# hsinnan75/MapCaller

Measured on AMD Instinct MI355X. Metric: reads/sec (150 bp PE vs GRCh38) at 1/2/4/8 MI355X; SAM CIGAR bit-exact, higher is better.
Workload: dtype u64/int32; 1 GPU; synthetic GRCh38-sized genome, 3100 Mbp (synthetic: GRCh38 is unavailable offline; repeat landscape in the detail record), 4000000 pairs x 150 bp PE per step per GPU (sub 0.005, ins 0.001, del 0.001 per base), -alg ksw2

## Files before the change

mapcaller_amd/csrc/mcx_ctx.h:

```cpp
#ifndef MCX_CTX_H
#define MCX_CTX_H
#include <hip/hip_runtime.h>
#include <algorithm>
#include <atomic>
#include <chrono>
#include <cmath>
#include <cstdio>
#include <cstdlib>
#include <cstring>
#include <string>
#include <type_traits>
#include <vector>

#include "../../include/mcx.h"
#include "mcx_dp.h"
#include "mcx_dp_lane2.h"
#include "mcx_simple.h"
#include "mcx_profile.h"
#include "mcx_internal.h"

using namespace mcx;

#define HIP_TRY(expr)                                                                                  \
    do {                                                                                               \
        hipError_t e_ = (expr);                                                                        \
        if (e_ != hipSuccess)                                                                          \
            return mcx_set_error(MCX_ERR_DEVICE, std::string(#expr) + ": " + hipGetErrorString(e_));   \
    } while (0)

template <typename F>
static inline hipError_t timed_wait(bool on, const char *what, int line, F &&f)
{
    if (!on) return f();
    const auto t0 = std::chrono::steady_clock::now();
    const hipError_t e = f();
    const double ms = std::chrono::duration<double, std::milli>(std::chrono::steady_clock::now() - t0).count();
    if (ms > 15) fprintf(stderr, "[mcx] %.1f ms in %s (line %d)\n", ms, what, line);
    return e;
}
extern std::atomic<size_t> g_dmalloc_bytes;
template <class T>
static int dmalloc(T **p, size_t n, int line = __builtin_LINE(), const char *file = __builtin_FILE())
{
    HIP_TRY(hipMalloc((void **)p, n * sizeof(T)));
    g_dmalloc_bytes += n * sizeof(T);
    static const bool log = getenv("MCX_ALLOC_LOG") != nullptr;
    if (log && n * sizeof(T) >= ((size_t)256 << 20)) fprintf(stderr, "[mcx alloc] %8.2f GB at %s:%d\n", (double)(n * sizeof(T)) / 1e9, file, line);
    return 0;
}

struct PairSel {
    const uint32_t *ids;
    const int32_t *est;
    uint32_t n;
};

static __device__ __forceinline__ uint32_t sel_pair(const PairSel &s, uint32_t local) { return s.ids ? s.ids[local] : local; }

constexpr int kCntPad = 64;
constexpr int kDpBuckets = 1024;

struct Knobs {
    bool timing = false, seed_one_base = false, dp_by_wave = false, dp_lane_always = false, late_reseed = false, no_work_order = false, no_simple = false,
         simple_no_dp = false, cluster_by_lane = false, rescue_in_line = false, build_by_lane = false, no_sums_cache = false, prof_by_column = false,
         tier1_hist = false, dp_hist = false, no_tier_overlap = false, no_late_overlap = false, no_prof_overlap = false, no_prepack = false, no_tier1_grow = false;
    int seed_fm_budget = 6, build_wave_limit = 0x7fffffff;
    uint32_t order_min = 16384u;
};

struct Tier {
    Caps caps;
    Layout lay;
    uint8_t *state = nullptr;
    uint32_t max_pairs = 0;
    uint32_t grow_to = 0;
};

enum { CNT_TASKS = 0, CNT_RESCUE = 1 * kCntPad, CNT_JOB0 = 2 * kCntPad, CNT_JOB1 = 3 * kCntPad, CNT_JOB2 = 4 * kCntPad, CNT_JOB3 = 5 * kCntPad,
       CNT_JOB4 = 6 * kCntPad, CNT_JOB5 = 7 * kCntPad, CNT_OV = 8 * kCntPad, CNT_LF = 9 * kCntPad, CNT_CELLS = 10 * kCntPad, CNT_UNSUP = 11 * kCntPad,
       CNT_QUEUE = 12 * kCntPad, CNT_EARLY = 13 * kCntPad, CNT_LATE = 14 * kCntPad, CNT_RTASK = 15 * kCntPad, CNT_RPLAN = 16 * kCntPad, CNT_RESCUE_N = 17 * kCntPad, CNT_RSEED = 18 * kCntPad,
       CNT_SIMPLE = 19 * kCntPad, CNT_EARLY_HITS = 20 * kCntPad, CNT_SIMPLE_LATER = 21 * kCntPad, CNT_SIMPLE_JOBS = 22 * kCntPad, CNT_N = 23 * kCntPad,
       CNT_ORDER = CNT_N, CNT_DP_SORT = CNT_ORDER + 16 * kCntPad, CNT_ALL = CNT_DP_SORT + 4 * kDpBuckets };
constexpr uint32_t kLateRoom = 2048;

struct RescueTask; struct RescueRes; struct RescuePlan;
struct PassRes {
    hipStream_t stream = nullptr;
    uint32_t *d_cnt = nullptr, *h_cnt = nullptr;
    uint2 *d_tasks = nullptr; uint32_t task_cap = 0;
    DpJob *d_jobs[kDpClasses] = {nullptr, nullptr, nullptr, nullptr, nullptr, nullptr}; uint32_t job_cap[kDpClasses] = {0, 0, 0, 0, 0, 0};
    uint32_t *d_rescue = nullptr; uint32_t rescue_cap = 0;
    uint32_t *d_kscratch = nullptr;
    RescueTask *d_rtasks = nullptr; RescueRes *d_rres = nullptr; Hit *d_rseeds = nullptr; RescuePlan *d_rplans = nullptr; uint32_t *d_rescue_n = nullptr;
    uint32_t rtask_cap = 0, rseed_cap = 0;
    uint8_t *d_dp_scratch[3] = {nullptr, nullptr, nullptr}; uint64_t dp_stride[3] = {0, 0, 0}; uint32_t dp_blocks[3] = {0, 0, 0};
    uint32_t *d_dp_lane = nullptr; uint32_t dp_lane_blocks = 0;
    uint32_t *d_dp_order[2] = {nullptr, nullptr};
    hipStream_t dp_stream[5] = {nullptr, nullptr, nullptr, nullptr, nullptr}; hipEvent_t dp_fork = nullptr, dp_join[5] = {nullptr, nullptr, nullptr, nullptr, nullptr};
    uint32_t *d_ov = nullptr; uint32_t ov_cap = 0;
    uint32_t *d_sel_ids = nullptr; int32_t *d_est = nullptr;
    hipEvent_t ev[12] = {nullptr, nullptr, nullptr, nullptr, nullptr, nullptr, nullptr, nullptr, nullptr, nullptr, nullptr, nullptr};
};

struct BatchRun {
    bool open = false, sums_valid = false, keys_out = false;
    ReadBatch rb; int paired = 0;
    uint32_t n_pairs = 0, n_chunks = 0, longest = 0;
    AlnRec *recs = nullptr; uint32_t *cig = nullptr;
    uint32_t cig_cap = 0, cig_words = 0;
    int64_t read_base = 0, mapped = 0;
    unsigned long long hs[3] = {0, 0, 0};
    std::vector<uint32_t> ok, ds;
    const uint32_t *d_ok = nullptr, *d_ds = nullptr;
    const uint64_t *d_sorted_keys = nullptr; uint64_t n_keys = 0; uint32_t n_sparse_keys = 0;
    std::chrono::steady_clock::time_point t0, t_begun; double ms_setup = 0;
    mcx_stats *stats = nullptr;
};
// ... 114 lines not shown
```

mapcaller_amd/csrc/mcx_pipeline.hip:

```cpp
#include "mcx_ctx.h"
#include <hipcub/hipcub.hpp>

static thread_local std::string g_err;
static int fail(int code, const std::string &msg) { g_err = msg; return code; }
int mcx_set_error(int code, const std::string &msg) { return fail(code, msg); }
extern "C" const char *mcx_last_error(void) { return g_err.c_str(); }
extern "C" int mcx_device_count(void)
{
    int n = 0;
    if (hipGetDeviceCount(&n) != hipSuccess) return 0;
    return n;
}

struct EndsLds { int64_t pos[kLdsEnds]; int32_t chr[kLdsEnds]; };

static __device__ __forceinline__ void stage_ends(IndexView &ix, EndsLds &l)
{
    if (ix.n_ends <= kLdsEnds) {
        for (int i = threadIdx.x; i < ix.n_ends; i += blockDim.x) { l.pos[i] = ix.end_pos[i]; l.chr[i] = ix.end_chr[i]; }
        __syncthreads();
        ix.end_pos = l.pos; ix.end_chr = l.chr;
    }
}

// ... 282 lines not shown
}

__global__ void __launch_bounds__(256) k_order_place(PairSel sel, const uint32_t *read_blocks, int nr, uint32_t *counts, uint32_t *order, const uint8_t *done)
{
    __shared__ uint32_t n_cls[kWorkClasses], at_cls[kWorkClasses];
    if (threadIdx.x < kWorkClasses) n_cls[threadIdx.x] = 0u;
    __syncthreads();
    const uint32_t base = blockIdx.x * (256u * kOrderTile);
    const int lane = threadIdx.x & 63;
    int cls[kOrderTile];
#pragma unroll
    for (int t = 0; t < kOrderTile; t++) {
        const uint32_t local = base + t * 256u + threadIdx.x;
        cls[t] = local < sel.n ? pair_work_class(sel, local, read_blocks, nr, done) : -1;
#pragma unroll
        for (int k = 0; k < kWorkClasses; k++) {
            const uint64_t m = __ballot(cls[t] == k);
            if (lane == 0 && m) atomicAdd(&n_cls[k], (uint32_t)__popcll(m));
        }
    }
    __syncthreads();
    if (threadIdx.x < kWorkClasses) {
        uint32_t first = 0;
        for (int k = 0; k < (int)threadIdx.x; k++) first += counts[k * kCntPad];
        const uint32_t mine = n_cls[threadIdx.x];
        at_cls[threadIdx.x] = first + (mine ? atomicAdd(counts + (8 + threadIdx.x) * kCntPad, mine) : 0u);
    }
    __syncthreads();
#pragma unroll
    for (int t = 0; t < kOrderTile; t++) {
        const uint32_t local = base + t * 256u + threadIdx.x;
#pragma unroll
        for (int k = 0; k < kWorkClasses; k++) {
            const uint64_t m = __ballot(cls[t] == k);
            uint32_t b = 0;
            if (lane == 0 && m) b = atomicAdd(&at_cls[k], (uint32_t)__popcll(m));
            b = __shfl(b, 0, 64);
            if (cls[t] == k) order[b + (uint32_t)__popcll(m & ((1ull << lane) - 1ull))] = local;
        }
    }
}

struct SimpleLater {
    uint32_t *pairs;
    SimpleJob *jobs;
    SimpleRes *res;
    uint32_t *job_list;
    uint32_t *n_pairs, *n_jobs;
    uint32_t cap;
};

template <bool NW, int MODE, bool DETAIL>
__global__ void __launch_bounds__(256) k_simple(Ctx cx, ReadBatch rb, uint32_t n_pairs, const int32_t *est, const uint32_t *read_blocks, AlnRec *recs, PairOut *pout,
                                                uint8_t *done, uint32_t *pool_over, uint32_t *n_done, SimpleLater sl)
{
    __shared__ EndsLds ends;
    __shared__ uint16_t cig_stage[256 * 2 * kSimpleRuns];
    __shared__ uint32_t job_stage[MODE == kDpCollect ? 3 * kSimpleJobs * 256 : 1];
    stage_ends(cx.ix, ends);
    const uint32_t slot = blockIdx.x * blockDim.x + threadIdx.x;
    const int nr = cx.pm.paired ? 2 : 1;
    uint16_t *stage = cig_stage + threadIdx.x;
    const uint32_t n_slots = MODE == kDpReplay ? min(*sl.n_pairs, sl.cap) : n_pairs;
    bool ok = slot < n_slots;
    const uint32_t pair = MODE == kDpReplay ? (ok ? sl.pairs[slot] : 0u) : slot;
    SimpleRead sr[2];
    int rl[2] = {0, 0};
    typename std::conditional<DETAIL, SimpleDetail, SimpleNoDetail>::type det;
    SimpleDpIo io;
    io.mode = MODE == kDpCollect && !sl.pairs ? kDpNone : MODE;
    io.jobs = MODE == kDpCollect ? job_stage + threadIdx.x : nullptr; io.job_stride = 256;
    io.res = MODE == kDpReplay ? sl.res + (uint64_t)slot * kSimpleJobs : nullptr;
    io.n = 0; io.read = 0;
    bool later = false;
    if (ok) {
        const PairState st = pair_state(cx.state, cx.lay, cx.caps, pair);
#pragma unroll
        for (int s = 0; s < 2; s++) {
            if (s < nr && ok) {
                const uint32_t r = pair * nr + s;
                const int nh = (int)(read_blocks[r] >> 20);
                rl[s] = (int)(rb.off[r + 1] - rb.off[r]);
                io.read = r;
                ok = nh >= 1 && nh <= kSimpleHits && !(cx.read_ext[r] >> 31);
                if (ok) {
                    if constexpr (DETAIL) { uint8_t *rec = cx.detail + (uint64_t)r * cx.dlay.stride; det.frags = (Frag *)(rec + sizeof(DetailHdr)); det.ops = rec + cx.dlay.off_ops; }
                    const int how = simple_read<NW, uint16_t>(cx.ix, cx.pm, rl[s], cx.packed + (uint64_t)r * cx.wpad, st.hits[s], nh, sr[s], stage + s * kSimpleRuns * 256, 256, io, det);
                    ok = how != kSimpleNo;
                    later = later || how == kSimpleLater;
                }
            }
        }
        if (ok && nr == 2) ok = simple_pair_ok(sr[0], sr[1], est[pair]);
    }
    if (MODE == kDpCollect) {
        const bool wait = ok && later;
        const uint32_t at = wave_reserve(sl.n_pairs, wait ? 1u : 0u);
        const bool kept = wait && at < sl.cap;
        const uint32_t jat = wave_reserve(sl.n_jobs, kept ? (uint32_t)io.n : 0u);
        if (kept) {
            sl.pairs[at] = pair;
            for (int k = 0; k < io.n; k++) {
                const uint32_t *w = job_stage + (3 * k) * 256 + threadIdx.x;
                sl.jobs[(uint64_t)at * kSimpleJobs + k] = simple_job_unpack(w[0], w[256], w[512], pair * (uint32_t)nr, nr);
                sl.job_list[jat + k] = at * kSimpleJobs + (uint32_t)k;
            }
            done[pair] = 2;
        }
        if (wait) ok = false;
        later = kept;
    }
    const uint32_t want = ok ? (uint32_t)sr[0].n_cig + (nr == 2 ? (uint32_t)sr[1].n_cig : 0u) : 0u;
    const uint32_t at = wave_reserve(cx.cig_pool_n, want);
    const uint64_t took = __ballot(ok);
    if ((threadIdx.x & 63) == 0 && took) atomicAdd(n_done, (uint32_t)__popcll(took));
    if (slot >= n_slots) return;
    if (ok && at + want > cx.cig_pool_cap) { atomicOr(pool_over, 1u); ok = false; }
    if (!later) done[pair] = ok ? 1 : 0;
    if (!ok) return;
    const uint32_t off[2] = {at, at + (uint32_t)sr[0].n_cig};
#pragma unroll
    for (int s = 0; s < 2; s++) {
        if (s >= nr) break;
        for (int k = 0; k < sr[s].n_cig; k++) cx.cig_pool[off[s] + k] = (uint32_t)stage[(s * kSimpleRuns + k) * 256];
    }
    AlnRec rec2[2];
    PairOut po;
    simple_pair(cx, nr == 2, sr[0], sr[nr - 1], rl[0], rl[nr - 1], est[pair], rec2, off, po);
    recs[(uint64_t)pair * nr] = rec2[0];
    if (nr == 2) recs[(uint64_t)pair * nr + 1] = rec2[1];
    pout[pair] = po;
    if constexpr (DETAIL) {
#pragma unroll
        for (int s = 0; s < 2; s++) {
            if (s >= nr) break;
            const DetailHdr d = simple_detail_hdr(cx.ix, nr == 2, s, sr[0], sr[nr - 1]);
            *(DetailHdr *)(cx.detail + ((uint64_t)pair * nr + s) * cx.dlay.stride) = d;
        }
    }
}

template <bool NW>
__global__ void __launch_bounds__(256) k_simple_dp(Ctx cx, SimpleLater sl)
{
    constexpr int W = 2 + kSimpleDp * LaneDir<16, NW>::words;
    __shared__ uint32_t words[W * 256];
    const uint32_t n = min(*sl.n_jobs, sl.cap * kSimpleJobs);
    LaneMem mem; mem.base = words; mem.stride = 256; mem.lane = threadIdx.x;
    for (uint32_t i = blockIdx.x * blockDim.x + threadIdx.x; i < n; i += gridDim.x * blockDim.x) {
        const uint32_t at = sl.job_list[i];
        const SimpleJob j = sl.jobs[at];
        sl.res[at] = simple_dp_job<NW>(cx.ix, j, cx.packed + (uint64_t)j.read * cx.wpad, mem);
    }
}

static __device__ __forceinline__ uint32_t listed_pairs(const PairSel &sel, const uint32_t *order_cnt)
{
    if (!order_cnt) return sel.n;
    uint32_t n = 0;
#pragma unroll
    for (int k = 0; k < kWorkClasses; k++) n += order_cnt[k * kCntPad];
    return n;
}

__global__ void __launch_bounds__(256) k_cluster(Ctx cx, ReadBatch rb, PairSel sel, RescueList rl, const uint32_t *read_blocks, EarlyList el, const uint32_t *order,
                                                 const uint32_t *order_cnt, int cls_lo, int cls_hi)
{
    __shared__ EndsLds ends;
    uint32_t first = 0, n_listed = listed_pairs(sel, order_cnt);
    if (order_cnt && order) {
        uint32_t at = 0;
        for (int k = 0; k < kWorkClasses; k++) { if (k == cls_lo) first = at; at += order_cnt[k * kCntPad]; if (k == cls_hi) n_listed = at; }
    }
    if (first + blockIdx.x * blockDim.x >= n_listed) return;
    stage_ends(cx.ix, ends);
    const uint32_t slot = first + blockIdx.x * blockDim.x + threadIdx.x;
    const bool in = slot < n_listed;
    const uint32_t local = in ? (order ? order[slot] : slot) : 0u;
    uint32_t need = 0, over = 0;
    if (in) {
        ReadRef rd[2];
// ... 678 lines not shown
    int n_cig[2] = {0, 0};
    uint8_t *detail2 = nullptr;
    if (active) {
        pair = sel_pair(sel, local);
        make_reads(cx, rb, pair, rd);
        st = pair_state(cx.state, cx.lay, cx.caps, local);
        h = *st.hdr;
        st.hdr = &h;
        detail2 = cx.detail ? cx.detail + (int64_t)pair * nr * cx.dlay.stride : nullptr;
        finish_scores(cx, st, rd, (DetailHdr *)detail2, n_cig, nullptr, stage, 256);
    }
    const uint32_t want = (uint32_t)(n_cig[0] + n_cig[1]);
    const uint32_t at = wave_reserve(cx.cig_pool_n, want);
    const bool own = active && !(h.flags & (kDispatched | kOvAny));
    int n_ext[2] = {0, 0}, n_extw[2] = {0, 0};
    uint32_t at_ext = 0, at_extw = 0;
    if (kMulti) {
        if (own) for (int s = 0; s < nr; s++) n_ext[s] = extra_lines(st, s, rd, &n_extw[s]);
        at_ext = wave_reserve(mo.cnt, (uint32_t)(n_ext[0] + n_ext[1]));
        at_extw = wave_reserve(mo.cnt + 1, (uint32_t)(n_extw[0] + n_extw[1]));
    }
    if (!active || (h.flags & kDispatched)) return;
    const bool fits = at + want <= cx.cig_pool_cap;
    if (!fits) atomicOr(pool_over, 1u);
    const uint32_t off[2] = {at, at + (uint32_t)n_cig[0]};
    finish_records(cx, st, rd, recs + (int64_t)pair * nr, fits ? cx.cig_pool : nullptr, off, n_cig, detail2, stage, 256);
    if (kMulti && own) {
        const bool room = at_ext + (uint32_t)(n_ext[0] + n_ext[1]) <= mo.rec_cap && at_extw + (uint32_t)(n_extw[0] + n_extw[1]) <= mo.word_cap;
        for (int s = 0; s < nr; s++) {
            const uint32_t ro = at_ext + (s ? (uint32_t)n_ext[0] : 0u), wo = at_extw + (s ? (uint32_t)n_extw[0] : 0u);
            mo.ref[(int64_t)pair * nr + s] = room || n_ext[0] + n_ext[1] == 0 ? make_uint4(ro, (uint32_t)n_ext[s], wo, (uint32_t)n_extw[s]) : make_uint4(0u, (uint32_t)n_ext[s] | kMxOver, 0u, 0u);
            if (room && n_ext[s]) emit_extra(cx, st, s, rd, mo.recs + ro, mo.cig + wo, wo);
        }
    }
    PairOut o;
    o.flags = h.flags; o.est = h.est; o.est_lo = h.est_lo; o.est_hi = h.est_hi;
    o.pair_dist = h.pair_dist; o.pair_ok = (int16_t)h.pair_ok; o.mapped = (int16_t)h.mapped;
    pout[pair] = o;
    if (h.flags & kOvAny) {
        const uint32_t at2 = atomicAdd(n_ov, 1u);
        if (at2 < ov_cap) ov_ids[at2] = pair;
    }
}

static Knobs knobs_read()
{
    Knobs k;
    auto on = [](const char *name) { return getenv(name) != nullptr; };
    k.timing = on("MCX_TIMING"); k.seed_one_base = on("MCX_SEED_ONE_BASE"); k.dp_by_wave = on("MCX_DP_BY_WAVE"); k.dp_lane_always = on("MCX_DP_LANE_ALWAYS");
    k.late_reseed = on("MCX_LATE_RESEED"); k.no_work_order = on("MCX_NO_WORK_ORDER"); k.no_simple = on("MCX_NO_SIMPLE"); k.simple_no_dp = on("MCX_SIMPLE_NO_DP");
    k.cluster_by_lane = on("MCX_CLUSTER_BY_LANE"); k.rescue_in_line = on("MCX_RESCUE_IN_LINE"); k.build_by_lane = on("MCX_BUILD_BY_LANE");
    k.no_sums_cache = on("MCX_NO_SUMS_CACHE"); k.prof_by_column = on("MCX_PROF_BY_COLUMN"); k.tier1_hist = on("MCX_TIER1_HIST"); k.dp_hist = on("MCX_DP_HIST");
    k.no_tier_overlap = on("MCX_NO_TIER_OVERLAP"); k.no_late_overlap = on("MCX_NO_LATE_OVERLAP"); k.no_prof_overlap = on("MCX_NO_PROF_OVERLAP"); k.no_tier1_grow = on("MCX_NO_TIER1_GROW");
    k.no_prepack = !on("MCX_PREPACK");
    if (const char *e = getenv("MCX_SEED_FM_BUDGET")) k.seed_fm_budget = std::max(1, atoi(e));
    if (const char *e = getenv("MCX_BUILD_WAVE_LIMIT")) k.build_wave_limit = atoi(e);
    if (const char *e = getenv("MCX_ORDER_MIN")) k.order_min = (uint32_t)std::max(1, atoi(e));
    return k;
}

constexpr uint32_t kPoutSel = 1u << 16;
static MultiOut multi_out(const mcx_ctx *c)
{
    MultiOut m;
    m.recs = c->mx.d_pool; m.cig = c->mx.d_pool_cig; m.cnt = c->mx.d_cnt; m.rec_cap = c->mx.rec_cap; m.word_cap = c->mx.word_cap; m.ref = c->mx.d_ref;
    return m;
}

extern "C" void mcx_opts_default(mcx_opts *o)
{
    o->alg = 0; o->max_pos_diff = 30; o->max_mismatch_rate = 0.05f; o->max_read_len = 256; o->max_batch_reads = 1 << 20;
}

static Caps tier0_caps()
{
    Caps c; c.hit_cap = 88; c.hit_seed = 56; c.cand_cap = 24; c.cand_seed = 12;
    c.frag_cap = 96; c.ops_cap = 2048; c.job_cap = 32;
    c.cig_cap = MCX_CIGAR_STRIDE; c.kmer_cap = 2048;
    return c;
}
static Caps tier1_caps(int rlen_max)
{
    Caps c;
    int seeds = rlen_max / (kMinSeedLength + 1) + 1;
    c.hit_cap = seeds * kOccThr + rlen_max / 8 + 16;
    c.cand_cap = c.hit_cap;
    c.hit_seed = c.hit_cap; c.cand_seed = c.cand_cap;
    c.frag_cap = 7 * c.hit_cap / 2 + 16;
    c.ops_cap = 96 * 1024; c.job_cap = 2048;
    c.cig_cap = MCX_CIGAR_STRIDE; c.kmer_cap = 4096;
    return c;
}

std::atomic<size_t> g_dmalloc_bytes(0);

static int ctx_fill(mcx_ctx *c, const mcx_index *idx, const mcx_opts &o);

extern "C" int mcx_ctx_create(const mcx_index *idx, const mcx_opts *opts, mcx_ctx **out)
{
    if (!idx || !out) return fail(MCX_ERR_ARG, "mcx_ctx_create: null argument");
    mcx_opts o;
    if (opts) o = *opts; else mcx_opts_default(&o);
    if (o.max_read_len < 32) o.max_read_len = 32;
    if (o.max_read_len > 1000) return fail(MCX_ERR_UNSUPPORTED, "max_read_len > 1000 is not supported");
    if (o.max_batch_reads < 2) o.max_batch_reads = 2;
    mcx_ctx *c = new mcx_ctx();
// ... 332 lines not shown
    HIP_TRY(hipMemsetAsync(R.d_cnt, 0, CNT_ALL * sizeof(uint32_t), s));
    SeedOut so; so.tasks = R.d_tasks; so.n_tasks = R.d_cnt + CNT_TASKS; so.task_cap = R.task_cap;
    so.read_ext = c->d_read_ext; so.read_blocks = c->d_read_blocks;
    so.packed = c->packed_now ? c->packed_now : c->d_packed; so.wpad = c->wpad; so.queue = R.d_cnt + CNT_QUEUE;
    so.src_state = nullptr; so.src_lay = c->tier[0].lay; so.src_caps = c->tier[0].caps;
    if (hits_from_tier0 && tier == 1 && cx.ix.sa_full && !kn.late_reseed) so.src_state = c->tier[0].state;
    RescueList rl; rl.ids = R.d_rescue; rl.n = R.d_cnt + CNT_RESCUE; rl.cap = R.rescue_cap;
    EarlyList el; el.ids = nullptr; el.est = nullptr; el.n = R.d_cnt + CNT_EARLY; el.cap = 0; el.n_hits = R.d_cnt + CNT_EARLY_HITS;
    if (early) { el.ids = c->t1.d_sel_ids; el.est = c->t1.d_est; el.cap = (uint32_t)c->max_reads; }
    const bool late = early && c->overlap_late;
    EarlyList ll; ll.ids = nullptr; ll.est = nullptr; ll.n = R.d_cnt + CNT_LATE; ll.cap = 0; ll.n_hits = R.d_cnt + CNT_EARLY_HITS;
    if (late) { ll.ids = c->t2.d_sel_ids; ll.est = c->t2.d_est; ll.cap = kLateRoom; }
    JobSinks sinks;
    for (int k = 0; k < kDpClasses; k++) { sinks.s[k].jobs = R.d_jobs[k]; sinks.s[k].count = R.d_cnt + CNT_JOB0 + k * kCntPad; sinks.s[k].cap = R.job_cap[k]; }
    sinks.unsupported = R.d_cnt + CNT_UNSUP;
    const unsigned pb = (sel.n + 255) / 256;
    int e = 0, rc2 = 0;
    if (timing) HIP_TRY(hipEventRecord(R.ev[e++], s));
    {
        const int pkw = packed_words(c->rlen_max);
        const int threads = pkw * 256 * 4 <= 48 * 1024 ? 256 : (pkw * 128 * 4 <= 48 * 1024 ? 128 : 64);
        const int rpl = seed_reads_per_lane((uint64_t)sel.n * nr);
        const unsigned blocks_s = std::min<unsigned>((sel.n * nr + threads * rpl - 1) / (threads * rpl), 4096u);
        k_seed<<<blocks_s, threads, (size_t)pkw * threads * 4, s>>>(cx, rb, sel, so, pkw, rpl, kn.seed_fm_budget);
#ifdef MCX_SEED_STATS
        if (tier == 0 && sel.n > 100000) {
            unsigned long long h[2][24];
            (void)hipStreamSynchronize(s);
            (void)hipMemcpyFromSymbol(h, HIP_SYMBOL(g_seed_hist), sizeof h);
            fprintf(stderr, "[k_seed] index blocks per read, by bit length of the count: reads");
            for (int k = 0; k < 12; k++) fprintf(stderr, " %llu", h[0][k]);
            fprintf(stderr, " | blocks");
            for (int k = 0; k < 12; k++) fprintf(stderr, " %llu", h[1][k]);
            fprintf(stderr, "\n");
            memset(h, 0, sizeof h);
            (void)hipMemcpyToSymbol(HIP_SYMBOL(g_seed_hist), h, sizeof h);
        }
#endif
    }
    if (timing) HIP_TRY(hipEventRecord(R.ev[e++], s));
    if (R.d_tasks) k_sa<<<4096, 256, 0, s>>>(cx, so, paired, R.d_cnt + CNT_LF);
    if (timing) HIP_TRY(hipEventRecord(R.ev[e++], s));
    const uint32_t *order = nullptr, *order_cnt = nullptr;
    bool split = false;
    if (tier == 0 && sel.n >= kn.order_min && c->d_order && !kn.no_work_order) {
        const bool no_simple = kn.no_simple;
        const uint8_t *done = nullptr;
        if (!no_simple && !sel.ids && cx.ix.sa_full && cx.packed) {
            SimpleLater sl; sl.pairs = kn.simple_no_dp ? nullptr : c->d_sl_pairs; sl.jobs = c->d_sl_jobs; sl.res = c->d_sl_res; sl.job_list = c->d_sl_list;
            sl.n_pairs = R.d_cnt + CNT_SIMPLE_LATER; sl.n_jobs = R.d_cnt + CNT_SIMPLE_JOBS; sl.cap = std::min<uint32_t>(c->sl_cap, std::max<uint32_t>(sel.n / 2, 1024u));
            const unsigned lb = (sl.cap + 255) / 256, jb = std::min<unsigned>((sl.cap * kSimpleJobs + 255) / 256, 3072u);
            auto launch = [&](auto nw, auto detail) {
                constexpr bool NW = decltype(nw)::value, DT = decltype(detail)::value;
                k_simple<NW, kDpCollect, DT><<<pb, 256, 0, s>>>(cx, rb, sel.n, sel.est, so.read_blocks, d_recs, c->d_pout, c->d_done, c->d_batch_flags + 2, R.d_cnt + CNT_SIMPLE, sl);
                if (sl.pairs) {
                    k_simple_dp<NW><<<jb, 256, 0, s>>>(cx, sl);
                    k_simple<NW, kDpReplay, DT><<<lb, 256, 0, s>>>(cx, rb, sel.n, sel.est, so.read_blocks, d_recs, c->d_pout, c->d_done, c->d_batch_flags + 2, R.d_cnt + CNT_SIMPLE, sl);
                }
            };
            if (cx.pm.use_nw) { if (cx.detail) launch(std::true_type(), std::true_type()); else launch(std::true_type(), std::false_type()); }
            else { if (cx.detail) launch(std::false_type(), std::true_type()); else launch(std::false_type(), std::false_type()); }
            done = c->d_done;
        }
        if (timing) HIP_TRY(hipEventRecord(R.ev[10], s));
        uint32_t *cls_cnt = R.d_cnt + CNT_ORDER;
        order_cnt = cls_cnt;
        const unsigned ob = (sel.n + 256 * kOrderTile - 1) / (256 * kOrderTile);
        k_order_count<<<ob, 256, 0, s>>>(sel, so.read_blocks, nr, cls_cnt, done);
        k_order_place<<<ob, 256, 0, s>>>(sel, so.read_blocks, nr, cls_cnt, c->d_order, done);
        order = c->d_order;
        if (timing) { HIP_TRY(hipEventRecord(R.ev[11], s)); split = true; }
    }
    const size_t cl_bytes = cluster_lds_bytes(cx.caps.hit_cap, cx.caps.cand_cap);
    if (tier == 1 && cl_bytes <= 60 * 1024 && !kn.cluster_by_lane) {
        const int small = std::min(kClusterSmall, cx.caps.hit_cap);
        k_cluster_wave<<<std::min<unsigned>(sel.n, 16384u), 64, cluster_lds_bytes(small, small), s>>>(cx, rb, sel, rl, so.read_blocks, -1, small, small, small);
        if (small < cx.caps.hit_cap)
            k_cluster_wave<<<std::min<unsigned>(sel.n, 8192u), 64, cl_bytes, s>>>(cx, rb, sel, rl, so.read_blocks, small, 1 << 30, cx.caps.hit_cap, cx.caps.cand_cap);
    } else k_cluster<<<pb, 256, 0, s>>>(cx, rb, sel, rl, so.read_blocks, el, order, order_cnt, 0, kWorkClasses - 1);
    if (early && c->h_early) k_publish_early<<<1, 64, 0, s>>>(R.d_cnt + CNT_EARLY, c->d_batch_flags + 3, c->d_early);
    if (early) HIP_TRY(hipEventRecord(c->ev_clustered, s));
    if (timing) HIP_TRY(hipEventRecord(R.ev[e++], s));
    const bool rescue_aside = paired && R.dp_stream[0] && !kn.rescue_in_line;
    hipStream_t rs = rescue_aside ? R.dp_stream[0] : s;
    if (rescue_aside) { HIP_TRY(hipEventRecord(R.dp_fork, s)); HIP_TRY(hipStreamWaitEvent(rs, R.dp_fork, 0)); }
    if (paired) {
        {
            RescueWork rw; rw.tasks = R.d_rtasks; rw.res = R.d_rres; rw.seeds = R.d_rseeds; rw.plans = R.d_rplans; rw.n_tasks = R.d_cnt + CNT_RTASK; rw.n_plans = R.d_cnt + CNT_RPLAN; rw.n_seeds = R.d_cnt + CNT_RSEED;
            rw.task_cap = R.rtask_cap; rw.seed_cap = R.rseed_cap; rw.ids_n = R.d_rescue_n; rw.n_ids_n = R.d_cnt + CNT_RESCUE_N;
            RescueList rn; rn.ids = R.d_rescue_n; rn.n = R.d_cnt + CNT_RESCUE_N; rn.cap = R.rescue_cap;
            const unsigned gb = std::min<unsigned>(std::max<unsigned>((sel.n + 255) / 256, 1u), 1024u);
            k_rescue_plan<<<gb, 256, 0, rs>>>(cx, rb, sel, rl, rw);
            if (tier == 0) k_rescue_eval<2048><<<4096, 256, 0, rs>>>(cx, rb, sel, rw);
            else k_rescue_eval<4096><<<4096, 256, 0, rs>>>(cx, rb, sel, rw);
            k_rescue_apply<<<gb, 256, 0, rs>>>(cx, rw);
            if (no_n_reads) {}
            else if (tier == 0) k_rescue<2048><<<256, kRescueThreads, 0, rs>>>(cx, rb, sel, rn, R.d_kscratch);
            else k_rescue<4096><<<256, kRescueThreads, 0, rs>>>(cx, rb, sel, rn, R.d_kscratch);
        }
    }
    const size_t bw_bytes = (size_t)6 * cx.caps.cand_cap * sizeof(int32_t);
    const bool build_wave = tier == 1 && bw_bytes <= 48 * 1024 && !kn.build_by_lane;
    const int build_wave_limit = kn.build_wave_limit;
    auto build = [&](int mode) {
        if (build_wave) k_build_wave<<<std::min<unsigned>(sel.n, 8192u), 64, bw_bytes, s>>>(cx, rb, sel, sinks, R.d_cnt + CNT_CELLS, R.d_cnt + CNT_UNSUP, mode, rl, build_wave_limit);
        else k_build<<<pb, 256, 0, s>>>(cx, rb, sel, sinks, R.d_cnt + CNT_CELLS, R.d_cnt + CNT_UNSUP, ll, order, order_cnt, mode, rl);
    };
    if (rescue_aside) {
        HIP_TRY(hipEventRecord(R.dp_join[0], rs));
        build(1);
// ... 1036 lines not shown
```

mapcaller_amd/csrc/mcx_simple.h:

```cpp
#ifndef MCX_SIMPLE_H
#define MCX_SIMPLE_H
#include "mcx_glue.h"
#include "mcx_dp_lane.h"

namespace mcx {

#ifndef MCX_SIMPLE_FAIL
#define MCX_SIMPLE_FAIL(code) return 0
#endif
#ifndef MCX_SIMPLE_NOTE
#define MCX_SIMPLE_NOTE(k, l) ((void)0)
#endif

constexpr int kSimpleHits = 4;
constexpr int kSimpleRuns = 12;
constexpr int kSimpleDp = 16;
constexpr int kSimpleJobs = 4;

struct SimpleJob { uint32_t read; uint16_t rp; uint8_t rl, gl; int64_t gp; };
struct SimpleCols {
    uint64_t w = 0; int len = 0, n = 0, mis = 0, switches = 0, cur = -1;
    MCX_HD bool wants_bases() const { return true; }
    MCX_HD void col(int kind, int differ) { w |= (uint64_t)kind << (2 * len); len++; if (kind == 0) { n++; mis += differ; } if (kind != cur) { cur = kind; switches++; } }
};
struct SimpleRes { uint64_t w; uint8_t len, n, mis, switches; uint8_t pad[4]; };
enum : int { kDpNone = 0, kDpCollect = 1, kDpReplay = 2 };
static inline MCX_HD SimpleJob simple_job_unpack(uint32_t w0, uint32_t w1, uint32_t w2, uint32_t first_read, int nr)
{
    SimpleJob j;
    j.rp = (uint16_t)(w0 & 0xFFFFu); j.rl = (uint8_t)((w0 >> 16) & 31u); j.gl = (uint8_t)((w0 >> 21) & 31u);
    j.read = nr == 2 ? (first_read & ~1u) | ((w0 >> 26) & 1u) : first_read;
    j.gp = (int64_t)((uint64_t)w1 | ((uint64_t)w2 << 32));
    return j;
}
struct SimpleDpIo {
    int mode;
    uint32_t *jobs;
    int job_stride;
    const SimpleRes *res;
    int n;
    uint32_t read;
};

template <bool NW> static inline MCX_HD LaneLayout simple_dp_layout()
{
    LaneLayout l; l.off_q = 0; l.off_edge = 0; l.off_dir = 2; l.rows = kSimpleDp; l.words = 2 + kSimpleDp * LaneDir<16, NW>::words; return l;
}

template <bool NW>
static inline MCX_HD SimpleRes simple_dp_job(const IndexView &ix, const SimpleJob &j, const uint32_t *codes, const LaneMem &mem)
{
    const bool rev = j.gp >= ix.G;
    const LaneLayout l = simple_dp_layout<NW>();
    const int rl_ = j.rl, gl_ = j.gl;
    mem.put(l.off_q, lane_query16(codes, j.rp, rl_, rev, 0));
    mem.put(l.off_q + 1, 0u);
    auto tgt16 = [&](int b0) -> uint32_t { return lane_target16(ix, j.gp, gl_, rev, b0); };
    SimpleCols sc;
    if (NW) { (void)lane_sweep_nw<16>(mem, l, rl_, gl_, tgt16); lane_walk_nw<16>(mem, l, rl_, gl_, tgt16, sc); }
    else { lane_sweep_ksw2<16>(mem, l, rl_, gl_, tgt16); lane_walk_ksw2<16>(mem, l, rl_, gl_, tgt16, sc); }
    SimpleRes r; r.w = sc.w; r.len = (uint8_t)sc.len; r.n = (uint8_t)sc.n; r.mis = (uint8_t)sc.mis; r.switches = (uint8_t)sc.switches;
    r.pad[0] = r.pad[1] = r.pad[2] = r.pad[3] = 0;
    return r;
}

constexpr int kSimpleFrags = 2 * kSimpleHits + 1;
struct SimpleNoDetail {
    static constexpr bool on = false;
    static constexpr int nf = 0, no = 0, fwd = 1;
    MCX_HD void frag(int, int, int64_t, int, int, int, int, int) {}
    MCX_HD int cols(uint64_t, int, int, int) { return 0; }
    MCX_HD void begin(bool) {}
    MCX_HD int frag0() const { return 0; }
};
struct SimpleDetail {
    static constexpr bool on = true;
    Frag *frags; uint8_t *ops; int nf, no, fwd;
    MCX_HD void begin(bool forward) { nf = 0; no = 0; fwd = forward ? 1 : 0; }
    MCX_HD int frag0() const { return fwd ? 0 : kSimpleFrags - nf; }
    MCX_HD void frag(int kind, int rp, int64_t gp, int rl, int gl, int ops_off, int ops_len, int meta)
    {
        Frag x; x.gPos = gp; x.rPos = rp; x.gLen = gl; x.rLen = rl; x.ops_off = ops_off; x.ops_len = ops_len; x.kind = (uint64_t)kind; x.meta = (uint64_t)meta;
        frags[fwd ? nf : kSimpleFrags - 1 - nf] = x;
        nf++;
    }
    MCX_HD int cols(uint64_t w, int len, int a, int b)
    {
        const int at = no;
        for (int j = a; j < b; j++) ops[no++] = (uint8_t)"MID"[(w >> (2 * (len - 1 - j))) & 3u];
        return at;
    }
};

struct SimpleRead {
    int64_t pd0;
    int64_t g_first;
    int64_t g_coord;
    int32_t score;
    int32_t fwd;
    int32_t n_cig;
    int32_t n_frags, n_ops, frag0;
};

enum : int { kSimpleNo = 0, kSimpleYes = 1, kSimpleLater = 2 };
template <bool NW, class CigT, class Det>
static inline MCX_HD int simple_read(const IndexView &ix, const Params &pm, int rlen, const uint32_t *codes, const Hit *hits, int n,
                                     SimpleRead &out, CigT *cig, int cig_stride, SimpleDpIo &io, Det &det)
{
    if (n < 1 || n > kSimpleHits || !codes) MCX_SIMPLE_FAIL(1);
    int64_t g[kSimpleHits], pd[kSimpleHits];
    int r[kSimpleHits], len[kSimpleHits];
    MCX_UNROLL
    for (int i = 0; i < kSimpleHits; i++) {
        if (i < n) { const Hit h = hits[i]; g[i] = h.gPos; r[i] = h.rPos; len[i] = h.len; pd[i] = h.gPos - h.rPos; if (pd[i] <= 0) MCX_SIMPLE_FAIL(2); }
        else { g[i] = 0; r[i] = 0x7fffffff; len[i] = 0; pd[i] = (int64_t)1 << 62; }
    }
    {
        int64_t sp[kSimpleHits], sg0 = 0;
        MCX_UNROLL
        for (int i = 0; i < kSimpleHits; i++) sp[i] = pd[i];
        {
            int64_t bp = sp[0]; int br = r[0]; sg0 = g[0];
            MCX_UNROLL
            for (int i = 1; i < kSimpleHits; i++) if (i < n && (pd[i] < bp || (pd[i] == bp && r[i] < br))) { bp = pd[i]; br = r[i]; sg0 = g[i]; }
            out.pd0 = bp;
        }
        auto cx2 = [](int64_t &a, int64_t &b) { if (a > b) { const int64_t t = a; a = b; b = t; } };
        cx2(sp[0], sp[1]); cx2(sp[2], sp[3]); cx2(sp[0], sp[2]); cx2(sp[1], sp[3]); cx2(sp[1], sp[2]);
        MCX_UNROLL
        for (int i = 1; i < kSimpleHits; i++) if (i < n && sp[i] - sp[i - 1] > pm.max_pos_diff) MCX_SIMPLE_FAIL(3);
        const int64_t g_end = boundary_of(ix, sg0);
        int score = 0;
        MCX_UNROLL
        for (int i = 0; i < kSimpleHits; i++) if (i < n) { if (g[i] > g_end) MCX_SIMPLE_FAIL(4); score += len[i]; }
        if (score <= (rlen >> 2)) MCX_SIMPLE_FAIL(5);
        if (score >= rlen && n > 1) MCX_SIMPLE_FAIL(6);
    }
    {
        auto cx4 = [&](int a, int b) {
            if (r[a] > r[b]) {
                const int64_t tg = g[a]; g[a] = g[b]; g[b] = tg;
                const int tr = r[a]; r[a] = r[b]; r[b] = tr;
                const int tl = len[a]; len[a] = len[b]; len[b] = tl;
            }
        };
        cx4(0, 1); cx4(2, 3); cx4(0, 2); cx4(1, 3); cx4(1, 2);
    }
    const int max_mm = (int)(rlen * pm.max_mm_rate);
    const int min_score = (int)(rlen * (1 - pm.max_mm_rate));
    int score = 0, mism = 0;
    int n_run = 0, run_len = 0, run_op = -1;
    uint32_t runs[kSimpleRuns];
    MCX_UNROLL
    for (int k = 0; k < kSimpleRuns; k++) runs[k] = 0;
    auto add = [&](int l, int op) {
        if (op != run_op) {
            if (run_len > 0) {
                const uint32_t w = ((uint32_t)run_len << 4) | (uint32_t)run_op;
                MCX_UNROLL
                for (int k = 0; k < kSimpleRuns; k++) if (k == n_run) runs[k] = w;
                n_run++;
            }
            run_op = op; run_len = 0;
        }
        run_len += l;
    };
    bool later = false, end_dropped = false;
// ... 71 lines not shown
        } else {
            const int rg = r0 - pr;
            const int64_t gg = g0 - pg;
            if (r0 <= prev_r || g0 <= prev_g || rg < 0 || gg < 0) MCX_SIMPLE_FAIL(10);
            if (rg > 0 && gg > 0) {
                if ((int64_t)rg != gg) { if (gg > kSimpleDp || !dp_gap(pr, pg, rg, (int)gg, 0)) { MCX_SIMPLE_NOTE(1, (int)(gg > rg ? gg : rg)); MCX_SIMPLE_FAIL(11); } }
                else if (!plain_gap(pr, pg, rg, 0)) MCX_SIMPLE_FAIL(12);
            } else if (rg > 0) { add(rg, 1); det.frag(kIns, pr, pg, rg, 0, 0, rg, 0); }
            else if (gg > 0) { if (gg >= 4096) MCX_SIMPLE_FAIL(13); add((int)gg, 2); det.frag(kDel, pr, pg, 0, (int)gg, 0, (int)gg, 0); }
        }
        score += len[i];
        add(len[i], 0);
        det.frag(kSimple, r0, g0, len[i], len[i], 0, 0, 0);
        prev_r = r0; prev_g = g0; pr = r0 + len[i]; pg = g0 + len[i];
    }
    if (pr < rlen) { if (!plain_gap(pr, pg, rlen - pr, 2)) MCX_SIMPLE_FAIL(14); pg += rlen - pr; }
    g_tail = pg;
    if (g_head < 0 || g_tail > ix.G2) MCX_SIMPLE_FAIL(15);
    {
        const int e1 = end_slot(ix, g_head), e2 = end_slot(ix, g_tail - 1);
        if (e1 < 0 || e2 < 0 || ix.end_pos[e1] != ix.end_pos[e2]) MCX_SIMPLE_FAIL(16);
    }
    if (later) return kSimpleLater;
    if (score == 0 || (score < min_score && mism > max_mm)) MCX_SIMPLE_FAIL(17);
    {
        const uint32_t w = ((uint32_t)run_len << 4) | (uint32_t)run_op;
        MCX_UNROLL
        for (int k = 0; k < kSimpleRuns; k++) if (k == n_run) runs[k] = w;
        n_run++;
    }
    if (n_run > kSimpleRuns) MCX_SIMPLE_FAIL(20);
    const int fwd = g_head + head_shift < ix.G ? 1 : 0;
    if (Det::on && fwd != det.fwd) MCX_SIMPLE_FAIL(21);
    MCX_UNROLL
    for (int k = 0; k < kSimpleRuns; k++) if (k < n_run) cig[(fwd ? k : n_run - 1 - k) * cig_stride] = (CigT)runs[k];
    out.score = score; out.fwd = fwd; out.n_cig = n_run;
    if (Det::on) { out.n_frags = det.nf; out.n_ops = det.no; out.frag0 = det.frag0(); }
    if (fwd) { out.g_first = g_head + head_shift; out.g_coord = g_head + head_shift; }
    else {
        int64_t last_g = 0;
        MCX_UNROLL
        for (int i = 0; i < kSimpleHits; i++) if (i == n - 1) last_g = (r[i] + len[i] < rlen) ? g[i] + len[i] : g[i];
        out.g_first = last_g; out.g_coord = g_tail - tail_shift - 1;
    }
    return kSimpleYes;
}

static inline MCX_HD bool simple_pair_ok(const SimpleRead &a, const SimpleRead &b, int est)
{
    return b.pd0 >= a.pd0 && b.pd0 - a.pd0 < (int64_t)est;
}

static inline MCX_HD bool simple_pair(const Ctx &cx, int paired, const SimpleRead &a, const SimpleRead &b, int rlen_a, int rlen_b, int est,
                                      AlnRec *rec2, const uint32_t cig_off[2], PairOut &po)
{
    const IndexView &ix = cx.ix;
    po.flags = 0; po.est = est; po.est_lo = 0; po.est_hi = 0x7fffffff; po.pair_dist = 0; po.pair_ok = 0; po.mapped = (int16_t)(paired ? 2 : 1); po.pad[0] = po.pad[1] = 0;
    int64_t d = 0;
    if (paired) {
        if (!simple_pair_ok(a, b, est)) return false;
        d = b.pd0 - a.pd0;
        po.est_lo = (int)(d + 1);
        const int64_t g1 = a.g_first, g2 = b.g_first;
        const int64_t dist = g2 > g1 ? g2 - g1 : g1 - g2;
        const bool inv = (g1 < ix.G && g2 >= ix.G) || (g1 >= ix.G && g2 < ix.G);
        if (dist != 0 && !inv && dist <= kMinTranslocationSize) { po.pair_ok = 1; po.pair_dist = (int)dist; }
    }
    const SimpleRead *rd2[2] = {&a, &b};
    const int rl[2] = {rlen_a, rlen_b};
    Coord k[2];
    MCX_UNROLL
    for (int s = 0; s < 2; s++) { if (s == 1 && !paired) break; k[s] = to_coord(ix, rd2[s]->g_coord); }
    MCX_UNROLL
    for (int s = 0; s < 2; s++) {
        if (s == 1 && !paired) break;
        const SimpleRead &me = *rd2[s];
        AlnRec o;
        o.pos = k[s].pos; o.chr = k[s].chr; o.mapq = 60; o.fwd = me.fwd;
        o.nm = rl[s] - me.score; o.as = me.score; o.xs = 0; o.n_cigar = me.n_cig; o.pad[0] = (int32_t)cig_off[s]; o.pad[1] = 0;
        if (paired) {
            int fl = s == 0 ? 0x41 : 0x81;
            if (s == 0) fl |= me.fwd ? 0x20 : 0x10; else fl |= me.fwd ? 0x10 : 0x20;
            o.flag = fl | 0x2;
            const int dist = (int)(k[1].pos - k[0].pos + (a.fwd ? rl[1] : 0 - rl[0]));
            o.tlen = s == 0 ? dist : 0 - dist;
            o.mate_pos = k[1 - s].pos; o.has_mate = 1;
        } else { o.flag = me.fwd ? 0 : 0x10; o.tlen = 0; o.mate_pos = 0; o.has_mate = 0; }
        rec2[s] = o;
    }
    return true;
}

static inline MCX_HD DetailHdr simple_detail_hdr(const IndexView &ix, int paired, int s, const SimpleRead &a, const SimpleRead &b)
{
    const SimpleRead &me = s == 0 ? a : b;
    DetailHdr d;
    d.type = 1; d.n_frags = me.n_frags; d.fwd = me.fwd; d.n_ops = me.n_ops; d.disc_kind = 0; d.frag0 = me.frag0; d.disc_g1 = d.disc_g2 = d.disc_dist = 0;
    if (s == 0 && paired) {
        const int64_t g1 = a.g_first, g2 = b.g_first, dist = g2 > g1 ? g2 - g1 : g1 - g2, G = ix.G;
        d.disc_g1 = g1; d.disc_g2 = g2; d.disc_dist = dist;
        if (dist != 0) {
            if (g1 < G && g2 >= G) d.disc_kind = 1;
            else if (g1 >= G && g2 < G) d.disc_kind = 2;
            else if (dist > kMinTranslocationSize) d.disc_kind = (g1 < G && g2 < G) ? 3 : 4;
        }
    }
    return d;
}

}
#endif
```

Measured before the change: 535.9 million reads/s.

## Let simple fast path handle multi-cluster reads via on-device cluster selection

Widens the simple-alignment fast path to accept reads with up to 8 seed hits, clustering them by diagonal on the device and pairing candidate clusters to pick a unique best pair. The chosen cluster's seeds are passed as a bitmask into simple_read, and the pair's estimate bounds are set from the cluster distances. More pairs should finish in the cheap path instead of falling through to full clustering and DP, at the cost of extra per-thread sorting and register pressure in k_simple. The old single-cluster behaviour remains available through an environment knob.

```diff
diff --git a/mapcaller_amd/csrc/mcx_ctx.h b/mapcaller_amd/csrc/mcx_ctx.h
--- a/mapcaller_amd/csrc/mcx_ctx.h
+++ b/mapcaller_amd/csrc/mcx_ctx.h
@@ -62,7 +62,7 @@
 
 struct Knobs {
     bool timing = false, seed_one_base = false, dp_by_wave = false, dp_lane_always = false, late_reseed = false, no_work_order = false, no_simple = false,
-         simple_no_dp = false, cluster_by_lane = false, rescue_in_line = false, build_by_lane = false, no_sums_cache = false, prof_by_column = false,
+         simple_no_dp = false, simple_one_cluster = false, cluster_by_lane = false, rescue_in_line = false, build_by_lane = false, no_sums_cache = false, prof_by_column = false,
          tier1_hist = false, dp_hist = false, no_tier_overlap = false, no_late_overlap = false, no_prof_overlap = false, no_prepack = false, no_tier1_grow = false;
     int seed_fm_budget = 6, build_wave_limit = 0x7fffffff;
     uint32_t order_min = 16384u;
diff --git a/mapcaller_amd/csrc/mcx_pipeline.hip b/mapcaller_amd/csrc/mcx_pipeline.hip
--- a/mapcaller_amd/csrc/mcx_pipeline.hip
+++ b/mapcaller_amd/csrc/mcx_pipeline.hip
@@ -358,7 +358,7 @@
 
 template <bool NW, int MODE, bool DETAIL>
 __global__ void __launch_bounds__(256) k_simple(Ctx cx, ReadBatch rb, uint32_t n_pairs, const int32_t *est, const uint32_t *read_blocks, AlnRec *recs, PairOut *pout,
-                                                uint8_t *done, uint32_t *pool_over, uint32_t *n_done, SimpleLater sl)
+                                                uint8_t *done, uint32_t *pool_over, uint32_t *n_done, SimpleLater sl, int one_cluster)
 {
     __shared__ EndsLds ends;
     __shared__ uint16_t cig_stage[256 * 2 * kSimpleRuns];
@@ -371,6 +371,7 @@
     bool ok = slot < n_slots;
     const uint32_t pair = MODE == kDpReplay ? (ok ? sl.pairs[slot] : 0u) : slot;
     SimpleRead sr[2];
+    SimpleSel sel; sel.mask[0] = sel.mask[1] = 0u; sel.est_lo = 0; sel.est_hi = 0x7fffffff;
     int rl[2] = {0, 0};
     typename std::conditional<DETAIL, SimpleDetail, SimpleNoDetail>::type det;
     SimpleDpIo io;
@@ -381,20 +382,28 @@
     bool later = false;
     if (ok) {
         const PairState st = pair_state(cx.state, cx.lay, cx.caps, pair);
+        int nh[2] = {0, 0};
+#pragma unroll
+        for (int s = 0; s < 2; s++) {
+            if (s >= nr) break;
+            const uint32_t r = pair * nr + s;
+            nh[s] = (int)(read_blocks[r] >> 20);
+            rl[s] = (int)(rb.off[r + 1] - rb.off[r]);
+            ok = ok && nh[s] >= 1 && nh[s] <= (one_cluster ? kSimpleHits : kSimpleIn) && !(cx.read_ext[r] >> 31);
+        }
+        if (ok && !one_cluster) {
+            const Hit *const hp[2] = {st.hits[0], st.hits[1]};
+            ok = simple_select(cx.ix, cx.pm, nr == 2, rl, hp, nh, est[pair], sel);
+        }
 #pragma unroll
         for (int s = 0; s < 2; s++) {
             if (s < nr && ok) {
                 const uint32_t r = pair * nr + s;
-                const int nh = (int)(read_blocks[r] >> 20);
-                rl[s] = (int)(rb.off[r + 1] - rb.off[r]);
                 io.read = r;
-                ok = nh >= 1 && nh <= kSimpleHits && !(cx.read_ext[r] >> 31);
-                if (ok) {
-                    if constexpr (DETAIL) { uint8_t *rec = cx.detail + (uint64_t)r * cx.dlay.stride; det.frags = (Frag *)(rec + sizeof(DetailHdr)); det.ops = rec + cx.dlay.off_ops; }
-                    const int how = simple_read<NW, uint16_t>(cx.ix, cx.pm, rl[s], cx.packed + (uint64_t)r * cx.wpad, st.hits[s], nh, sr[s], stage + s * kSimpleRuns * 256, 256, io, det);
-                    ok = how != kSimpleNo;
-                    later = later || how == kSimpleLater;
-                }
+                if constexpr (DETAIL) { uint8_t *rec = cx.detail + (uint64_t)r * cx.dlay.stride; det.frags = (Frag *)(rec + sizeof(DetailHdr)); det.ops = rec + cx.dlay.off_ops; }
+                const int how = simple_read<NW, uint16_t>(cx.ix, cx.pm, rl[s], cx.packed + (uint64_t)r * cx.wpad, st.hits[s], nh[s], sr[s], stage + s * kSimpleRuns * 256, 256, io, det, sel.mask[s]);
+                ok = how != kSimpleNo;
+                later = later || how == kSimpleLater;
             }
         }
         if (ok && nr == 2) ok = simple_pair_ok(sr[0], sr[1], est[pair]);
@@ -432,7 +441,7 @@
     }
     AlnRec rec2[2];
     PairOut po;
-    simple_pair(cx, nr == 2, sr[0], sr[nr - 1], rl[0], rl[nr - 1], est[pair], rec2, off, po);
+    simple_pair(cx, nr == 2, sr[0], sr[nr - 1], rl[0], rl[nr - 1], est[pair], rec2, off, po, one_cluster ? nullptr : &sel);
     recs[(uint64_t)pair * nr] = rec2[0];
     if (nr == 2) recs[(uint64_t)pair * nr + 1] = rec2[1];
     pout[pair] = po;
@@ -1217,6 +1226,7 @@
     k.cluster_by_lane = on("MCX_CLUSTER_BY_LANE"); k.rescue_in_line = on("MCX_RESCUE_IN_LINE"); k.build_by_lane = on("MCX_BUILD_BY_LANE");
     k.no_sums_cache = on("MCX_NO_SUMS_CACHE"); k.prof_by_column = on("MCX_PROF_BY_COLUMN"); k.tier1_hist = on("MCX_TIER1_HIST"); k.dp_hist = on("MCX_DP_HIST");
     k.no_tier_overlap = on("MCX_NO_TIER_OVERLAP"); k.no_late_overlap = on("MCX_NO_LATE_OVERLAP"); k.no_prof_overlap = on("MCX_NO_PROF_OVERLAP"); k.no_tier1_grow = on("MCX_NO_TIER1_GROW");
+    k.simple_one_cluster = on("MCX_SIMPLE_ONE_CLUSTER");
     k.no_prepack = !on("MCX_PREPACK");
     if (const char *e = getenv("MCX_SEED_FM_BUDGET")) k.seed_fm_budget = std::max(1, atoi(e));
     if (const char *e = getenv("MCX_BUILD_WAVE_LIMIT")) k.build_wave_limit = atoi(e);
@@ -1655,10 +1665,10 @@
             const unsigned lb = (sl.cap + 255) / 256, jb = std::min<unsigned>((sl.cap * kSimpleJobs + 255) / 256, 3072u);
             auto launch = [&](auto nw, auto detail) {
                 constexpr bool NW = decltype(nw)::value, DT = decltype(detail)::value;
-                k_simple<NW, kDpCollect, DT><<<pb, 256, 0, s>>>(cx, rb, sel.n, sel.est, so.read_blocks, d_recs, c->d_pout, c->d_done, c->d_batch_flags + 2, R.d_cnt + CNT_SIMPLE, sl);
+                k_simple<NW, kDpCollect, DT><<<pb, 256, 0, s>>>(cx, rb, sel.n, sel.est, so.read_blocks, d_recs, c->d_pout, c->d_done, c->d_batch_flags + 2, R.d_cnt + CNT_SIMPLE, sl, kn.simple_one_cluster ? 1 : 0);
                 if (sl.pairs) {
                     k_simple_dp<NW><<<jb, 256, 0, s>>>(cx, sl);
-                    k_simple<NW, kDpReplay, DT><<<lb, 256, 0, s>>>(cx, rb, sel.n, sel.est, so.read_blocks, d_recs, c->d_pout, c->d_done, c->d_batch_flags + 2, R.d_cnt + CNT_SIMPLE, sl);
+                    k_simple<NW, kDpReplay, DT><<<lb, 256, 0, s>>>(cx, rb, sel.n, sel.est, so.read_blocks, d_recs, c->d_pout, c->d_done, c->d_batch_flags + 2, R.d_cnt + CNT_SIMPLE, sl, kn.simple_one_cluster ? 1 : 0);
                 }
             };
             if (cx.pm.use_nw) { if (cx.detail) launch(std::true_type(), std::true_type()); else launch(std::true_type(), std::false_type()); }
diff --git a/mapcaller_amd/csrc/mcx_simple.h b/mapcaller_amd/csrc/mcx_simple.h
--- a/mapcaller_amd/csrc/mcx_simple.h
+++ b/mapcaller_amd/csrc/mcx_simple.h
@@ -13,6 +13,8 @@
 #endif
 
 constexpr int kSimpleHits = 4;
+constexpr int kSimpleIn = 8;
+constexpr int kSimpleCands = 4;
 constexpr int kSimpleRuns = 12;
 constexpr int kSimpleDp = 16;
 constexpr int kSimpleJobs = 4;
@@ -92,6 +94,109 @@
     }
 };
 
+struct SimpleCands { int n; int64_t pd0[kSimpleCands]; int score[kSimpleCands]; uint32_t seeds[kSimpleCands]; };
+struct SimpleSel { uint32_t mask[2]; int est_lo, est_hi; };
+
+static inline MCX_HD int simple_cluster(const IndexView &ix, const Params &pm, int rlen, const Hit *hits, int n, SimpleCands &c)
+{
+    c.n = 0;
+    if (n < 1 || n > kSimpleIn) MCX_SIMPLE_FAIL(24);
+    int64_t pd[kSimpleIn];
+    uint32_t w[kSimpleIn];
+    int m = 0;
+    MCX_UNROLL
+    for (int i = 0; i < kSimpleIn; i++) {
+        pd[i] = (int64_t)1 << 62; w[i] = 0xFFFFFFFFu;
+        if (i < n) {
+            const Hit h = hits[i];
+            if ((uint32_t)h.rPos >= 4096u || (uint32_t)h.len >= 4096u) MCX_SIMPLE_FAIL(24);
+            if (h.gPos - h.rPos > 0) { pd[i] = h.gPos - h.rPos; w[i] = ((uint32_t)h.rPos << 15) | ((uint32_t)h.len << 3) | (uint32_t)i; m++; }
+        }
+    }
+    if (m == 0) MCX_SIMPLE_FAIL(25);
+    {
+        auto cx = [&](int a, int b) {
+            if (pd[a] > pd[b] || (pd[a] == pd[b] && w[a] > w[b])) { const int64_t t = pd[a]; pd[a] = pd[b]; pd[b] = t; const uint32_t u = w[a]; w[a] = w[b]; w[b] = u; }
+        };
+        cx(0, 2); cx(1, 3); cx(4, 6); cx(5, 7); cx(0, 4); cx(1, 5); cx(2, 6); cx(3, 7); cx(0, 1); cx(2, 3); cx(4, 5); cx(6, 7);
+        cx(2, 4); cx(3, 5); cx(1, 4); cx(3, 6); cx(1, 2); cx(3, 4); cx(5, 6);
+    }
+    int nc = 0, score = (int)((w[0] >> 3) & 4095u), thr = rlen >> 2, count = 1;
+    uint32_t seeds = 1u << (w[0] & 7u);
+    int64_t head_pd = pd[0], pd_prev = pd[0];
+    int64_t g_end = boundary_of(ix, pd[0] + (int64_t)(w[0] >> 15));
+    MCX_UNROLL
+    for (int j = 1; j <= kSimpleIn; j++) {
+        if (j > m) continue;
+        const bool last = j == m;
+        const int jj = j < kSimpleIn ? j : 0;
+        const int64_t pdj = last ? ix.G2 : pd[jj];
+        const int64_t gj = last ? ix.G2 : pd[jj] + (int64_t)(w[jj] >> 15);
+        const int lj = last ? 0 : (int)((w[jj] >> 3) & 4095u);
+        int64_t d = pdj - pd_prev;
+        pd_prev = pdj;
+        if (d < 0) d = -d;
+        if (gj > g_end || d > pm.max_pos_diff) {
+            if (score > thr) {
+                if (thr < (score >> 1)) thr = score >> 1;
+                if (score >= rlen && count > 1) MCX_SIMPLE_FAIL(26);
+                if (nc >= kSimpleCands) MCX_SIMPLE_FAIL(27);
+                MCX_UNROLL
+                for (int k = 0; k < kSimpleCands; k++) if (k == nc) { c.pd0[k] = head_pd; c.score[k] = score; c.seeds[k] = seeds; }
+                nc++;
+            }
+            if (!last) { g_end = boundary_of(ix, gj); score = lj; seeds = 1u << (w[jj] & 7u); count = 1; head_pd = pdj; }
+        } else { score += lj; seeds |= 1u << (w[jj] & 7u); count++; }
+    }
+    if (nc == 0) MCX_SIMPLE_FAIL(25);
+    c.n = nc;
+    return nc;
+}
+
+static inline MCX_HD bool simple_select(const IndexView &ix, const Params &pm, int paired, const int *rlen, const Hit *const *hits, const int *n, int est, SimpleSel &sel)
+{
+    SimpleCands a, b;
+    sel.mask[0] = sel.mask[1] = 0; sel.est_lo = 0; sel.est_hi = 0x7fffffff;
+    if (!simple_cluster(ix, pm, rlen[0], hits[0], n[0], a)) return false;
+    if (paired) {
+        if (!simple_cluster(ix, pm, rlen[1], hits[1], n[1], b)) return false;
+        int64_t max_lt = -1, min_ge = 0x7fffffff;
+        int pick[kSimpleCands], sum[kSimpleCands], top = 0;
+        MCX_UNROLL
+        for (int i = 0; i < kSimpleCands; i++) {
+            pick[i] = -1; sum[i] = 0;
+            if (i >= a.n) continue;
+            int ps = 0;
+            MCX_UNROLL
+            for (int j = 0; j < kSimpleCands; j++) {
+                if (j >= b.n) continue;
+                const int64_t d = b.pd0[j] - a.pd0[i];
+                if (d < 0) continue;
+                if (d < (int64_t)est) { if (d > max_lt) max_lt = d; if (b.score[j] > ps) { pick[i] = j; ps = b.score[j]; } }
+                else if (d < min_ge) min_ge = d;
+            }
+            if (pick[i] >= 0) { sum[i] = a.score[i] + ps; if (sum[i] > top) top = sum[i]; }
+        }
+        if (top == 0) MCX_SIMPLE_FAIL(28);
+        int paired_n = 0, p2 = -1;
+        MCX_UNROLL
+        for (int i = 0; i < kSimpleCands; i++) if (pick[i] >= 0 && sum[i] == top) { paired_n++; sel.mask[0] = a.seeds[i]; p2 = pick[i]; }
+        if (paired_n != 1) MCX_SIMPLE_FAIL(29);
+        MCX_UNROLL
+        for (int j = 0; j < kSimpleCands; j++) if (j == p2) sel.mask[1] = b.seeds[j];
+        sel.est_lo = (int)(max_lt + 1); sel.est_hi = (int)min_ge;
+    } else {
+        int best = 0, live = 0;
+        MCX_UNROLL
+        for (int i = 0; i < kSimpleCands; i++) if (i < a.n && a.score[i] > best) best = a.score[i];
+        MCX_UNROLL
+        for (int i = 0; i < kSimpleCands; i++) if (i < a.n && a.score[i] == best) { live++; sel.mask[0] = a.seeds[i]; }
+        if (live != 1) MCX_SIMPLE_FAIL(29);
+    }
+    if (__builtin_popcount(sel.mask[0]) > kSimpleHits || __builtin_popcount(sel.mask[1]) > kSimpleHits) MCX_SIMPLE_FAIL(30);
+    return true;
+}
+
 struct SimpleRead {
     int64_t pd0;
     int64_t g_first;
@@ -105,14 +210,15 @@
 enum : int { kSimpleNo = 0, kSimpleYes = 1, kSimpleLater = 2 };
 template <bool NW, class CigT, class Det>
 static inline MCX_HD int simple_read(const IndexView &ix, const Params &pm, int rlen, const uint32_t *codes, const Hit *hits, int n,
-                                     SimpleRead &out, CigT *cig, int cig_stride, SimpleDpIo &io, Det &det)
-{
+                                     SimpleRead &out, CigT *cig, int cig_stride, SimpleDpIo &io, Det &det, uint32_t take = 0u)
+{
+    if (take) n = __builtin_popcount(take);
     if (n < 1 || n > kSimpleHits || !codes) MCX_SIMPLE_FAIL(1);
     int64_t g[kSimpleHits], pd[kSimpleHits];
     int r[kSimpleHits], len[kSimpleHits];
     MCX_UNROLL
     for (int i = 0; i < kSimpleHits; i++) {
-        if (i < n) { const Hit h = hits[i]; g[i] = h.gPos; r[i] = h.rPos; len[i] = h.len; pd[i] = h.gPos - h.rPos; if (pd[i] <= 0) MCX_SIMPLE_FAIL(2); }
+        if (i < n) { const Hit h = hits[take ? __builtin_ctz(take) : i]; take &= take - 1u; g[i] = h.gPos; r[i] = h.rPos; len[i] = h.len; pd[i] = h.gPos - h.rPos; if (pd[i] <= 0) MCX_SIMPLE_FAIL(2); }
         else { g[i] = 0; r[i] = 0x7fffffff; len[i] = 0; pd[i] = (int64_t)1 << 62; }
     }
     {
@@ -290,7 +396,7 @@
 }
 
 static inline MCX_HD bool simple_pair(const Ctx &cx, int paired, const SimpleRead &a, const SimpleRead &b, int rlen_a, int rlen_b, int est,
-                                      AlnRec *rec2, const uint32_t cig_off[2], PairOut &po)
+                                      AlnRec *rec2, const uint32_t cig_off[2], PairOut &po, const SimpleSel *sel = nullptr)
 {
     const IndexView &ix = cx.ix;
     po.flags = 0; po.est = est; po.est_lo = 0; po.est_hi = 0x7fffffff; po.pair_dist = 0; po.pair_ok = 0; po.mapped = (int16_t)(paired ? 2 : 1); po.pad[0] = po.pad[1] = 0;
@@ -299,6 +405,7 @@
         if (!simple_pair_ok(a, b, est)) return false;
         d = b.pd0 - a.pd0;
         po.est_lo = (int)(d + 1);
+        if (sel) { po.est_lo = sel->est_lo; po.est_hi = sel->est_hi; }
         const int64_t g1 = a.g_first, g2 = b.g_first;
         const int64_t dist = g2 > g1 ? g2 - g1 : g1 - g2;
         const bool inv = (g1 < ix.G && g2 >= ix.G) || (g1 >= ix.G && g2 < ix.G);
```

New measurement: 541.9 million reads/s, median of 3. About the same (+1.1%).
